# chenhaoxing/DiffUTE

Measured on AMD Instinct MI355X. Metric: 512x512 50-step denoise images/sec, higher is better.
Workload: dtype bf16; 1 GPU; SD2-inpaint UNet 50-step DDIM denoise loop, 512x512 px, batch 4 per GPU, glyph context [B,577,1024], ctx K/V cached per image (BASELINE configs[1]); VAE encode/decode not in the timed region; global_batch=4, denoise_steps=50, parallelism=replicas x1 (no collective), weights=random-init SD2-inpainting shapes (865,925,124 params), bf16 packed

## Files before the change

diffute_amd/_cabi.py:

```python
import ctypes
import os
from ctypes import c_char_p, c_float, c_int, c_int64, c_size_t, c_void_p, POINTER

_LIB_DIR = os.path.join(os.path.dirname(os.path.abspath(__file__)), "lib")
_LIB_PATH = os.environ.get("DIFFUTE_HIP_LIB") or os.path.join(_LIB_DIR, "libdiffute_hip.so")
_LIB_PATH_F16 = os.environ.get("DIFFUTE_HIP_LIB_F16") or os.path.join(_LIB_DIR, "libdiffute_hip_f16.so")
_lib = None
_lib_f16 = None
_exclusive = None
_last_elem = "bf16"


class XfChainDesc(ctypes.Structure):
    _fields_ = [
        ("M", c_int), ("C", c_int), ("x", c_void_p), ("ldx", c_int), ("res", c_void_p), ("ldres", c_int),
        ("w0", c_void_p), ("b0", c_void_p), ("h_out", c_void_p), ("ldh", c_int), ("w1", c_void_p),
        ("c1", c_void_p), ("c2", c_void_p), ("y", c_void_p), ("ldy", c_int), ("wf1", c_void_p),
        ("wf2", c_void_p), ("bf2", c_void_p), ("wpo", c_void_p), ("bpo", c_void_p), ("xres", c_void_p), ("ldxres", c_int),
        ("eps", c_float), ("dbg", c_int), ("timing", c_void_p), ("colstats", c_void_p), ("cs_rows", c_int),
        ("gn_st", c_void_p), ("gn_gamma", c_void_p), ("gn_beta", c_void_p), ("gn_groups", c_int), ("gn_rows", c_int), ("gn_eps", c_float),
    ]


class GemmDesc(ctypes.Structure):
# ... 85 lines not shown
    "dmx_test_transpose_bf16": (c_int, [_P, c_int, _P, c_int, c_int, c_int, _P]),
    "dmx_test_transpose_batch": (c_int, [_P, c_int, _P, c_size_t, _P]),
    "dmx_test_add_bf16": (c_int, [_P, c_int, _P, c_int, _P, c_int, c_int, c_int, _P]),
    "dmx_test_softmax_rows": (c_int, [_P, c_int, _P, c_int, c_int, c_int, c_float, _P]),
    "dmx_test_softmax_bwd_rows": (c_int, [_P, c_int, _P, c_int, _P, c_int, c_int, c_int, c_float, _P]),
    "dmx_test_pointwise_small_fwd": (c_int, [_P, c_int, _P, c_int, _P, _P, c_int, c_int, c_int, c_int, c_int, _P]),
    "dmx_test_pointwise_small_bwd_workspace_bytes": (c_size_t, [c_int, c_int, c_int]),
    "dmx_test_pointwise_small_bwd": (c_int, [_P, c_int, _P, c_int, _P, c_int, _P, c_int, _P, c_int, _P, c_int, c_int, c_int, _P, c_size_t, _P]),
    "dmx_test_linear_small_bwd": (c_int, [_P, c_int, _P, c_int, _P, c_int, _P, c_int, _P, c_int, _P, c_int, c_int, c_int, c_int, c_int, c_int, _P]),
    "dmx_test_slice_cast": (c_int, [_P, c_int, _P, c_int, c_int, c_int, _P]),
    "dmx_test_mode_bwd": (c_int, [_P, c_int, _P, c_int, c_int, _P]),
    "dmx_test_bf16_to_f32_rows": (c_int, [_P, c_int, _P, c_int, c_int, _P]),
    "dmx_conv_gemm_workspace_bytes": (c_size_t, [POINTER(GemmDesc)]),
    "dmx_conv_gemm": (c_int, [POINTER(GemmDesc), _P, c_size_t, _P]),
    "dmx_conv_gemm_rowstats_tiles": (c_int, [POINTER(GemmDesc)]),
    "dmx_conv_gemm_colstats_ok": (c_int, [POINTER(GemmDesc)]),
    "dmx_set_gn_producer_stats": (c_int, [c_int]),
    "dmx_conv3x3_gn_supported": (c_int, [POINTER(HaloConvDesc)]),
    "dmx_conv3x3_gn_workspace_bytes": (c_size_t, [POINTER(HaloConvDesc)]),
    "dmx_conv3x3_gn": (c_int, [POINTER(HaloConvDesc), _P, c_size_t, _P]),
    "dmx_colstats": (c_int, [_P, c_int, c_int, c_int, c_int, _P, _P]),
    "dmx_skinny_conv_supported": (c_int, [POINTER(SkinnyDesc)]),
    "dmx_skinny_conv_workspace_bytes": (c_size_t, [POINTER(SkinnyDesc)]),
    "dmx_skinny_conv": (c_int, [POINTER(SkinnyDesc), _P, c_size_t, _P]),
    "dmx_skinny_pack": (c_int, [_P, c_int, _P, c_int, c_int, POINTER(c_int), POINTER(c_int), POINTER(c_int), POINTER(c_int), _P]),
    "dmx_set_skinny": (c_int, [c_int]),
    "dmx_set_halo_conv": (c_int, [c_int]),
    "dmx_set_halo_ws": (c_int, [c_int]),
    "dmx_set_halo_peers": (c_int, [c_int]),
    "dmx_set_attn_balanced": (c_int, [c_int]),
    "dmx_attention_fwd_v_balanced_workspace_bytes": (c_size_t, [c_int, c_int, c_int, c_int]),
    "dmx_attention_fwd_v_balanced": (c_int, [c_void_p, c_int, c_void_p, c_int, c_void_p, c_int, c_int, c_void_p, c_int, c_int, c_int, c_int, c_int, c_float,
                                             c_void_p, c_size_t, c_void_p]),
    "dmx_set_defer_reduce": (c_int, [c_int]),
    "dmx_set_exclusive_device": (c_int, [c_int]),
    "dmx_get_exclusive_device": (c_int, []),
    "dmx_plan_epoch": (c_int, []),
    "dmx_xf_chain_ok": (c_int, [c_int, c_int]),
    "dmx_xf_chain": (c_int, [POINTER(XfChainDesc), c_int, _P]),
    "dmx_set_xf_chain": (c_int, [c_int]),
    "dmx_set_weight_prefetch": (c_int, [c_int]),
    "dmx_groupnorm_from_stats": (c_int, [_P, c_int, _P, c_int, c_int, c_int, c_int, c_int, c_int, _P, _P, c_float, c_int, _P, _P, _P, c_int, _P]),
    "dmx_conv_wgrad_workspace_bytes": (c_size_t, [POINTER(GemmDesc), c_int]),
    "dmx_conv_wgrad": (c_int, [POINTER(GemmDesc), _P, c_int, _P, c_int, _P, c_size_t, _P]),
    "dmx_colsum_workspace_bytes": (c_size_t, [c_int, c_int, c_int]),
    "dmx_colsum": (c_int, [_P, c_int, c_int, c_int, c_int, _P, c_int, c_int, _P, c_size_t, _P]),
    "dmx_groupnorm_workspace_bytes": (c_size_t, [c_int, c_int, c_int]),
    "dmx_groupnorm": (c_int, [_P, c_int, _P, c_int, c_int, c_int, c_int, c_int, c_int, _P, _P, c_float, c_int, _P, c_int, _P, c_size_t, _P]),
    "dmx_groupnorm_train": (c_int, [_P, c_int, _P, c_int, c_int, c_int, c_int, c_int, c_int, _P, _P, c_float, c_int, _P, c_int, _P, _P, c_size_t, _P]),
    "dmx_groupnorm_bwd_workspace_bytes": (c_size_t, [c_int, c_int, c_int]),
    "dmx_groupnorm_bwd": (c_int, [_P, c_int, _P, c_int, c_int, c_int, c_int, c_int, c_int, _P, _P, c_int, _P,
                                  _P, c_int, _P, c_int, _P, c_int, _P, c_int, _P, c_int, _P, _P, c_int, _P, c_size_t, _P]),
    "dmx_layernorm_bwd_workspace_bytes": (c_size_t, [c_int, c_int]),
    "dmx_layernorm_bwd": (c_int, [_P, c_int, _P, c_int, _P, _P, c_int, _P, c_int, _P, _P, c_int, c_int, c_int, c_float, _P, c_size_t, _P]),
    "dmx_geglu_fwd": (c_int, [_P, c_int, _P, c_int, c_int, c_int, _P]),
    "dmx_geglu_bwd": (c_int, [_P, c_int, _P, c_int, _P, c_int, c_int, c_int, _P]),
    "dmx_layernorm": (c_int, [_P, c_int, _P, c_int, _P, _P, c_int, c_int, c_float, _P]),
    "dmx_attention_fwd": (c_int, [_P, c_int, _P, c_int, c_int, _P, c_int, c_int, _P, c_int, c_int, c_int, c_int, c_int, c_float, _P]),
    "dmx_attention_fwd_v": (c_int, [_P, c_int, _P, c_int, _P, c_int, c_int, _P, c_int, c_int, c_int, c_int, c_int, c_float, _P]),
    "dmx_attention_wide": (c_int, [_P, c_int, _P, c_int, _P, c_int, c_int, _P, c_int, c_int, c_int, c_int, c_int, c_float, _P]),
    "dmx_attention_fwd_train": (c_int, [_P, c_int, _P, c_int, _P, c_int, c_int, _P, c_int, _P, c_int, c_int, c_int, c_int, c_float, _P]),
    "dmx_attention_bwd_workspace_bytes": (c_size_t, [c_int, c_int, c_int]),
    "dmx_attention_bwd": (c_int, [_P, c_int, _P, c_int, _P, c_int, c_int, _P, _P, c_int, _P, _P, c_int, _P, c_int, _P, c_int,
                                  c_int, c_int, c_int, c_int, c_float, _P, c_size_t, _P]),
    "dmx_timestep_embedding": (c_int, [_P, c_int, _P, c_int, c_int, _P, _P]),
    "dmx_linear_small": (c_int, [_P, c_int, _P, c_int, _P, _P, c_int, c_int, c_int, c_int, c_int, _P]),
# ... 235 lines not shown
```

diffute_amd/csrc/attention.hip:

```cpp
#include "common.h"
#include "kernels.h"
#include "attention_d64.h"
#include <stdlib.h>

#define KROW 72
#define VROW 68
#define VRS 192
#define KT_BYTES (64 * KROW * 2)
#define VT_BYTES (64 * VRS)

#define DMX_TR8(V, A, O0, O1, O2, O3, O4, O5, O6, O7)                                                     \
  asm volatile("ds_read_b64_tr_b16 %0, %8 offset:%9\n\tds_read_b64_tr_b16 %1, %8 offset:%10\n\t"          \
               "ds_read_b64_tr_b16 %2, %8 offset:%11\n\tds_read_b64_tr_b16 %3, %8 offset:%12\n\t"         \
               "ds_read_b64_tr_b16 %4, %8 offset:%13\n\tds_read_b64_tr_b16 %5, %8 offset:%14\n\t"         \
               "ds_read_b64_tr_b16 %6, %8 offset:%15\n\tds_read_b64_tr_b16 %7, %8 offset:%16"              \
               : "=&v"(V[0]), "=&v"(V[1]), "=&v"(V[2]), "=&v"(V[3]), "=&v"(V[4]), "=&v"(V[5]), "=&v"(V[6]), "=&v"(V[7]) \
               : "v"(A), "i"(O0), "i"(O1), "i"(O2), "i"(O3), "i"(O4), "i"(O5), "i"(O6), "i"(O7) : "memory")


template <bool VROWMAJOR, int R, int NW, int PROBE = 0>
__global__ __launch_bounds__(64 * NW, R == 2 ? 2 : (NW == 4 ? 2 : 3)) void dmx_attn_d64_kernel(const AttnArgs p) {
  constexpr int NT = 64 * NW, SL = 512 / NT;
  constexpr bool DMA = VROWMAJOR;
  constexpr int KTB = DMA ? 64 * 128 : KT_BYTES, VTB = DMA ? 64 * 128 : VT_BYTES;
// ... 526 lines not shown
    const float inv = 1.0f / l_tot;
    const int qrow = q0 + lr;
#ifdef DMX_ATTN_TIMING
    if (p.lse && lane == 0) {
      float* d = p.lse + ((size_t)((blockIdx.z * gridDim.y + blockIdx.y) * gridDim.x + blockIdx.x) * 4 + wave) * 4;
      d[0] = (float)tm_top; d[1] = (float)tm_slots; d[2] = (float)tm_wait; d[3] = (float)tm_bar;
    }
#else
    if (p.lse && qrow < p.Sq && lh == 0) p.lse[((size_t)b * p.H + h) * p.Sq + qrow] = m_run * sl2 + log2f(l_tot);
#endif
    if (qrow < p.Sq) {
      bf16* op = p.o + ((size_t)b * p.Sq + qrow) * p.ldo + h * 64 + 4 * lh;
#pragma unroll
      for (int dt = 0; dt < 2; ++dt)
#pragma unroll
        for (int g = 0; g < 4; ++g) {
          u32x2 pk = {pack_bf2(o[dt][4 * g] * inv, o[dt][4 * g + 1] * inv),
                      pack_bf2(o[dt][4 * g + 2] * inv, o[dt][4 * g + 3] * inv)};
          *(u32x2*)(op + 32 * dt + 8 * g) = pk;
        }
    }
  }
}

#endif

int dmx_attention_launch(const AttnArgs& a, hipStream_t stream) {
  DMX_REQUIRE(a.B > 0 && a.H > 0 && a.Sq > 0 && a.Skv > 0, "attention: empty problem");
  DMX_REQUIRE(a.kv_rows >= a.Skv, "attention: kv_rows=%d < Skv=%d", a.kv_rows, a.Skv);
  DMX_REQUIRE(a.ldq % 8 == 0 && a.ldk % 8 == 0 && a.ldo % 4 == 0, "attention: strides must be multiples of 8 (ldq=%d ldk=%d)", a.ldq, a.ldk);
  dim3 grid(cdiv(a.Sq, 128), a.H, a.B);
  if (a.v) {
    DMX_REQUIRE(a.ldv % 8 == 0, "attention: ldv=%d must be a multiple of 8", a.ldv);
#ifdef DMX_ATTN_PIPE
#ifndef DMX_ATTN_PIPE_MIN
#define DMX_ATTN_PIPE_MIN 1
#endif
    if (a.Skv >= DMX_ATTN_PIPE_MIN) {
      hipLaunchKernelGGL(dmx_attn_d64_pipe_kernel, grid, dim3(256), 0, stream, a);
      dmx_profile_note_symbol("dmx_attn_d64_pipe_kernel(AttnArgs)");
      return dmx_check_launch("dmx_attn_d64_pipe_kernel");
    }
#endif
#ifdef DMX_PROBES
#define PB(N) else if (pb == N) hipLaunchKernelGGL((dmx_attn_d64_kernel<true, 1, 4, N>), grid, dim3(256), 0, stream, a);
    if (const int pb = getenv("DMX_ATTN_PROBE_BITS") ? atoi(getenv("DMX_ATTN_PROBE_BITS")) : 0; pb == 0) hipLaunchKernelGGL((dmx_attn_d64_kernel<true, 1, 4>), grid, dim3(256), 0, stream, a);
    PB(1) PB(2) PB(4) PB(8) PB(16) PB(32) PB(96) PB(3) PB(7) PB(24) PB(31) PB(127) PB(120)
#undef PB
#else
    hipLaunchKernelGGL((dmx_attn_d64_kernel<true, 1, 4>), grid, dim3(256), 0, stream, a);
#endif
    dmx_profile_note_symbol("void dmx_attn_d64_kernel<true, 1, 4, 0>(AttnArgs)");
  } else {
    grid = dim3(cdiv(a.Sq, 128), a.H, a.B);
    DMX_REQUIRE(a.vt && a.ldvt % 8 == 0 && a.skv_stride % 8 == 0, "attention: V^T strides must be multiples of 8 (ldvt=%d skv_stride=%d)", a.ldvt, a.skv_stride);
    DMX_REQUIRE(a.skv_stride >= (a.Skv + 7) / 8 * 8, "attention: skv_stride=%d < Skv=%d rounded to 8", a.skv_stride, a.Skv);
    hipLaunchKernelGGL((dmx_attn_d64_kernel<false, 1, 4>), grid, dim3(256), 0, stream, a);
  }
  return dmx_check_launch("dmx_attn_d64_kernel");
}
```

diffute_amd/csrc/exec.hip:

```cpp
#include <stdarg.h>
#include <stdio.h>
#include <string.h>
#include "exec.h"
#include <vector>

static thread_local char g_err[512] = "";
void dmx_set_error(const char* fmt, ...) {
  va_list ap; va_start(ap, fmt); vsnprintf(g_err, sizeof(g_err), fmt, ap); va_end(ap);
}
const char* dmx_get_error() { return g_err; }
static int* g_dev_err = nullptr;
int* dmx_dev_err_words() {
  static bool tried = false;
  if (!tried) {
    tried = true;
    void* p = nullptr;
    if (hipHostMalloc(&p, 64, hipHostMallocMapped | hipHostMallocCoherent) == hipSuccess && p) { memset(p, 0, 64); g_dev_err = (int*)p; }
    else (void)hipGetLastError();
  }
  return g_dev_err;
}
int dmx_poll_device_error() {
  volatile int* e = g_dev_err;
  if (!e || !e[0]) return DMX_OK;
  const int k = e[0], blk = e[2], d0 = e[3], d1 = e[4], d2 = e[5];
  if (k == DMX_DEVK_HALO_PEER)
    dmx_set_error("device error: conv3x3_gn (halo conv) block %d gave up after 40 ms waiting for the K-split slab of peer %d of tile slot %d (splits %d) - "
                  "the blocks of a tile were not co-resident (CUs taken by another stream?); the result of that launch is invalid", blk, d1, d0, d2);
  else if (k == DMX_DEVK_STREAMK_HELPER)
    dmx_set_error("device error: stream-K GEMM block %d (tile %d) gave up after 40 ms waiting for the partial sums of helper block %d - "
                  "the blocks of the launch were not co-resident; the result of that launch is invalid", blk, d0, d1);
  else if (k == DMX_DEVK_SKINNY_PEER)
    dmx_set_error("device error: weight-streaming conv (skinny.hip) block %d gave up after 40 ms waiting for the partial tile of K slice %d of output tile %d (slices %d) - "
                  "the blocks of a tile were not co-resident (CUs taken by another stream?); the result of that launch is invalid", blk, d1, d0, d2);
  else if (k == DMX_DEVK_ATTN_PEER)
    dmx_set_error("device error: attention (balanced schedule) slot %d gave up after 40 ms waiting for the partial (O, m, l) record of slot %d for query block %d (%d slots) - "
                  "the slots in front of it did not run; the result of that launch is invalid", blk, d0, d1, d2);
  else
    dmx_set_error("device error %d raised by block %d (%d, %d, %d)", k, blk, d0, d1, d2);
  e[0] = 0;
  for (int i = 2; i < 8; ++i) e[i] = 0;
  __atomic_thread_fence(__ATOMIC_SEQ_CST);
  e[1] = 0;
  return DMX_ERR_DEVICE;
}
extern "C" int dmx_device_error(void) { return dmx_poll_device_error(); }
int dmx_check_launch(const char* what) {
  hipError_t e = hipGetLastError();
  if (e != hipSuccess) { dmx_set_error("launch of %s failed: %s", what, hipGetErrorString(e)); return DMX_ERR_HIP; }
  const int rc = dmx_poll_device_error();
  if (rc) {
    char first[400]; strncpy(first, dmx_get_error(), sizeof(first) - 1); first[sizeof(first) - 1] = 0;
    dmx_set_error("%s [surfaced at the launch check of %s, which itself was enqueued correctly; the walk it belongs to is abandoned]", first, what ? what : "?");
  }
  return rc;
}

static int g_plan_sw[DMX_SW_COUNT] = {1, 1, 1, 1, 1, 1, 1, 0, 1, 1, 1};
void dmx_plan_switch(int slot, int value) { if (slot >= 0 && slot < DMX_SW_COUNT) g_plan_sw[slot] = value; }
void dmx_plan_epoch_bump() { ++g_plan_sw[DMX_SW_OVERRIDES]; }
extern "C" int dmx_plan_epoch(void) {
  unsigned h = 2166136261u;
  for (int i = 0; i < DMX_SW_COUNT; ++i) h = (h ^ (unsigned)g_plan_sw[i]) * 16777619u;
  return (int)(h & 0x7fffffffu);
}

namespace {
struct ProfRec { hipEvent_t a, b; int cls; double flops, bytes; char tag[96]; char sym[112]; };
struct ProfSym { char sym[112]; int cls; double n, ms, flops, bytes; };
std::vector<ProfSym> g_prof_syms;
bool g_prof_on = false;
std::vector<ProfRec> g_prof;
char g_prof_path[512] = "";
}
ProfScope::ProfScope(ProfClass c, hipStream_t s, double flops, double bytes, const char* tag) {
  if (!g_prof_on) return;
  ProfRec r; r.cls = c; r.flops = flops; r.bytes = bytes; r.tag[0] = 0; r.sym[0] = 0;
  if (tag) { strncpy(r.tag, tag, sizeof(r.tag) - 1); r.tag[sizeof(r.tag) - 1] = 0; }
  if (hipEventCreate(&r.a) != hipSuccess || hipEventCreate(&r.b) != hipSuccess) return;
  (void)hipEventRecord(r.a, s);
  slot = (int)g_prof.size(); g_prof.push_back(r);
  stream_ = s;
}
ProfScope::~ProfScope() { if (slot >= 0) (void)hipEventRecord(g_prof[slot].b, stream_); }

bool dmx_profile_active() { return g_prof_on; }
void dmx_profile_note_symbol(const char* sym) {
  if (!g_prof_on || g_prof.empty() || !sym) return;
  strncpy(g_prof.back().sym, sym, sizeof(g_prof.back().sym) - 1); g_prof.back().sym[sizeof(g_prof.back().sym) - 1] = 0;
}
extern "C" int dmx_profile_begin(void) {
// ... 473 lines not shown
static int g_xf_chain = 1;
extern "C" int dmx_set_xf_chain(int on) { const int old = g_xf_chain; g_xf_chain = on; dmx_plan_switch(DMX_SW_XF_CHAIN, on); return old; }
bool Exec::chain_ok(const Tn& x) const { return (g_xf_chain & 3) && !f32 && x.ld == x.C && ((g_xf_chain & 3) > 1 ? dmx_xf_chain_supported(x.rows(), x.C) : dmx_xf_chain_pays(x.rows(), x.C)); }
bool Exec::chain_gn_fold(const Tn& x) const { return !(g_xf_chain & 4) && !f32 && x.cst != nullptr && (x.H * x.W) % 64 == 0 && x.ld == x.C; }
void Exec::chain_stats(XfChainArgs& a, Tn& y) {
  if (rc || f32 || !dmx_halo_conv_enabled() || !g_gn_producer_stats || (y.H * y.W) % 64) return;
  if (!dmx_conv_halo_wants_stats(y.H, y.W, g_halo_conv != 1)) return;
  a.colstats = stat_slice(y.B, y.C);
  if (!a.colstats) return;
  a.cs_rows = y.H * y.W; y.cst = a.colstats;
}
void Exec::xf_chain(int mode, XfChainArgs& a) {
  const long cc = (long)a.C * a.C * 2;
  note(a.w0, cc);
  if (mode == 0) note(a.w1, cc);
  else if (mode == 2) note(a.w1, 3 * cc);
  else { note(a.wf1, 8 * cc); note(a.wf2, 4 * cc); note(a.wpo, cc); }
  peek(a.pf, a.pf_bytes, 4);
  if (dry || rc) return;
  rc = dmx_xf_chain_launch(a, mode, stream);
}

void Exec::attention(const bf16* q, int ldq, const bf16* k, int ldk, const bf16* v, int ldv, int kv_rows,
                     bf16* o, int ldo, int B, int H, int Sq, int Skv, float scale, bool kv_static) {
#ifdef DMX_PROBES
  static const int kv_pf = [] { const char* e = getenv("DMX_PF_KV"); return e ? atoi(e) : 1; }();
#else
  constexpr int kv_pf = 1;
#endif
  if (kv_static && kv_pf) note(k, (long)B * kv_rows * ldk * 2);
  AttnArgs a{};
  a.q = q; a.ldq = ldq; a.k = k; a.ldk = ldk; a.kv_rows = kv_rows; a.v = v; a.ldv = ldv;
  a.o = o; a.ldo = ldo; a.B = B; a.H = H; a.Sq = Sq; a.Skv = Skv; a.scale = scale;
  const int sk_slots = f32 ? 0 : dmx_attention_balanced_slots(a);
  void* sk_ws = nullptr;
  if (sk_slots) {
    constexpr size_t POOL = 64 * 1024;
    if (!flag_pool) {
      flag_pool = (int*)raw(POOL * sizeof(int)); flag_cap = POOL; flag_used = 0;
      if (!zero_pool(flag_pool, POOL * sizeof(int), 2)) return;
    }
    const size_t n = align_up((size_t)sk_slots, 64);
    const size_t pb = dmx_attention_balanced_part_bytes(a);
    if (flag_used + n <= flag_cap) { a.sk_flags = flag_pool + flag_used; flag_used += n; sk_ws = raw(pb); a.sk_part = (float*)sk_ws; }
  }
  struct Rel { Workspace& w; void* p; ~Rel() { if (p) w.release(p); } } rel{ws, sk_ws};
  if (dry || rc) return;
  if (f32) {
    rc = dmx_attention_f32_launch((const float*)q, ldq, (const float*)k, ldk, (const float*)v, ldv, kv_rows, (float*)o, ldo, B, H, Sq, Skv, scale, stream);
    return;
  }
  {
#ifdef DMX_PROBES
    static const int attn_pf = [] { const char* e = getenv("DMX_PF_ATTN"); return e ? atoi(e) : 1; }();
#else
    constexpr int attn_pf = 1;
#endif
    if (attn_pf) peek(a.pf, a.pf_bytes, 4);
  }
  char tag[96]; snprintf(tag, sizeof(tag), "B=%d H=%d Sq=%d Skv=%d", B, H, Sq, Skv);
  ProfScope ps(PROF_ATTN, stream, 4.0 * B * H * (double)Sq * Skv * 64.0, 2.0 * 64.0 * B * H * (2.0 * Sq + 2.0 * Skv), tag);
  rc = a.sk_part ? dmx_attention_balanced_launch(a, stream) : dmx_attention_launch(a, stream);
}

void Exec::tap(const Tn& t) {
  if (!taps) return;
  flush(t);
// ... 88 lines not shown
```

diffute_amd/csrc/kernels.h:

```cpp
#pragma once
#include <vector>
#include "common.h"

enum ProfClass { PROF_GEMM128 = 0, PROF_GEMM64 = 1, PROF_SPLITK = 2, PROF_ATTN = 3, PROF_GNORM = 4, PROF_LNORM = 5,
                 PROF_OTHER = 6, PROF_GEMM256 = 7, PROF_WGRAD = 8, PROF_GEMM256WS = 9,
                 PROF_GEMM_CFG0 = 10 , PROF_XFCHAIN = 26 , PROF_HALO = 27 , PROF_SKINNY = 28 , PROF_NCLASS = 29 };
int n_cus();
enum DmxPlanSwitch { DMX_SW_EXCLUSIVE = 0, DMX_SW_GN_STATS, DMX_SW_DEFER, DMX_SW_HALO, DMX_SW_PREFETCH, DMX_SW_XF_CHAIN, DMX_SW_HALO_WS, DMX_SW_OVERRIDES, DMX_SW_SKINNY, DMX_SW_HALO_PEERS, DMX_SW_ATTN_BALANCED, DMX_SW_COUNT };
void dmx_plan_switch(int slot, int value);
void dmx_plan_epoch_bump();
extern "C" int dmx_plan_epoch(void);
int dmx_exclusive_device();
void dmx_profile_note_symbol(const char* sym);
struct ProfScope {
  ProfScope(ProfClass c, hipStream_t s, double flops, double bytes, const char* tag = nullptr);
  ~ProfScope();
  int slot = -1;
  hipStream_t stream_ = nullptr;
};

struct GemmArgs {
  const bf16* x0; const bf16* x1;
  int ldx0, ldx1;
  int cx0;
  int direct;
  int IH, IW, OH, OW;
  int stride, pad, ups, ksize;
  int ups2, M4; long long w_phase_stride;
  int Cin;
  int Ktaps;
  const bf16* s0; const bf16* s1; int lds0, lds1, cs0;
  const bf16* w; int ldw;
  int M, N, K;
  const float* bias;
  const float* rowbias;
  int rows_per_group, ldrb;
  const bf16* res; int ldres;
  void* out; int ldo; int out_f32; int geglu;
  int act;
  int force_tn, force_splitk;
  int group_m;
// ... 171 lines not shown
  bf16* y; int ldy;
  const bf16* wf1;
  const bf16* wf2; const float* bf2;
  const bf16* wpo; const float* bpo;
  const bf16* xres; int ldxres;
  float eps;
  int dbg; long long* timing;
  long long* colstats; int cs_rows;
  const void* pf[4]; int pf_bytes[4];
  const long long* gn_st; const float* gn_gamma; const float* gn_beta; int gn_groups; int gn_rows; float gn_eps;
};
bool dmx_xf_chain_supported(int M, int C);
bool dmx_xf_chain_pays(int M, int C);
int dmx_xf_chain_launch(const XfChainArgs& a, int mode, hipStream_t stream);

struct AttnArgs {
  const bf16* q; int ldq;
  const bf16* k; int ldk;
  int kv_rows;
  const bf16* vt; int ldvt;
  const bf16* v; int ldv;
  int skv_stride;
  bf16* o; int ldo;
  int B, H, Sq, Skv;
  float scale;
  float* lse;
  const void* pf[4]; int pf_bytes[4];
  float* sk_part; int* sk_flags; int* err;
};
int dmx_attention_launch(const AttnArgs& a, hipStream_t stream);
int dmx_attention_balanced_slots(const AttnArgs& a);
size_t dmx_attention_balanced_part_bytes(const AttnArgs& a);
int dmx_attention_balanced_launch(AttnArgs a, hipStream_t stream);

struct AttnWideArgs {
  const bf16* q; int ldq;
  const bf16* k; int ldk;
  const bf16* v; int ldv;
  int kv_rows;
  bf16* o; int ldo;
  int B, Sq, Skv, D;
  float scale;
  const bf16* zeros;
};
bool dmx_attention_wide_supported(int D);
int dmx_attention_wide_launch(AttnWideArgs a, hipStream_t stream);

struct AttnBwdArgs {
  const bf16* q; int ldq; const bf16* k; int ldk; const bf16* v; int ldv; int kv_rows;
  const bf16* o; const bf16* dout; int ldo;
  const float* lse;
  float* delta;
  bf16* dq; int lddq; bf16* dk; int lddk; bf16* dv; int lddv;
  int B, H, Sq, Skv; float scale;
};
size_t dmx_attn_bwd_ws_bytes(int B, int H, int Sq);
int dmx_attention_bwd_launch(const AttnBwdArgs& a, hipStream_t stream);

struct GemmF32Args {
  const float* x0; const float* x1; int ldx0, ldx1, cx0, direct;
  int IH, IW, OH, OW, stride, pad, ups, ksize, Cin, Ktaps;
  const float* s0; const float* s1; int lds0, lds1, cs0;
  const float* w; int ldw; int M, N, K;
  const float* bias; const float* bias2; const float* rowbias; int rows_per_group, ldrb;
  const float* res; int ldres;
  float* out; int ldo; int geglu, act;
// ... 72 lines not shown
```

include/diffute_hip.h:

```cpp
#ifndef DIFFUTE_HIP_H
#define DIFFUTE_HIP_H

#include <stddef.h>
#include <stdint.h>

#ifdef __cplusplus
extern "C" {
#endif

#define DMX_OK 0
#define DMX_ERR_ARG (-1)
#define DMX_ERR_HIP (-2)
#define DMX_ERR_UNSUPPORTED (-3)
#define DMX_ERR_WORKSPACE (-4)

typedef void* dmx_stream_t;
typedef struct dmx_unet dmx_unet;
typedef struct dmx_vae dmx_vae;

int dmx_version(void);
const char* dmx_last_error(void);
int dmx_device_error(void);
int dmx_test_raise_device_error(int code, dmx_stream_t stream);
int dmx_test_occupy_cus(int blocks, long long ticks, dmx_stream_t stream);
const char* dmx_element_type(void);

int dmx_test_transpose_bf16(const void* in, int ldin, void* out, int ldout, int R, int C, dmx_stream_t stream);
typedef struct dmx_test_tr_job { const void* in; int ldin; void* out; int ldout; int R, C; } dmx_test_tr_job;
int dmx_test_transpose_batch(const dmx_test_tr_job* h_jobs, int njobs, void* table, size_t table_bytes, dmx_stream_t stream);
int dmx_test_add_bf16(const void* a, int lda, const void* b, int ldb, void* out, int ldo, int rows, int C, dmx_stream_t stream);
int dmx_test_softmax_rows(const float* s, int lds, void* p, int ldp, int rows, int n, float scale, dmx_stream_t stream);
int dmx_test_softmax_bwd_rows(const void* p, int ldp, const float* dp, int lddp, void* ds, int ldds, int rows, int n, float scale, dmx_stream_t stream);
int dmx_test_pointwise_small_fwd(const void* x, int ldx, const void* w, int ldw, const float* bias, void* y, int ldy, int M, int Cin, int Cout,
                                 int out_f32, dmx_stream_t stream);
size_t dmx_test_pointwise_small_bwd_workspace_bytes(int M, int Cin, int Cout);
int dmx_test_pointwise_small_bwd(const void* x, int ldx, const float* dy, int lddy, const void* w, int ldw, void* dx, int lddx,
                                 float* dw, int lddw, float* db, int M, int Cin, int Cout, void* workspace, size_t workspace_bytes, dmx_stream_t stream);
int dmx_test_linear_small_bwd(const float* x, int ldx, const float* dy, int lddy, const void* w, int ldw, float* dw, int lddw, float* db, int db_stride,
                              float* dx, int lddx, int B, int N, int K, int silu_in, int accumulate, dmx_stream_t stream);
int dmx_test_slice_cast(const float* in, int ldin, void* out, int ldo, int M, int C, dmx_stream_t stream);
int dmx_test_mode_bwd(const void* dz, int lddz, float* dmom, int M, int C, dmx_stream_t stream);
int dmx_test_bf16_to_f32_rows(const void* in, int ldin, float* out, int M, int C, dmx_stream_t stream);


typedef struct dmx_gemm_desc {
  const void* x0; const void* x1;
  int ldx0, ldx1, cx0;
  int direct;
  int IH, IW, OH, OW;
  int stride, pad, ups, ksize;
  int Cin;
  int Ktaps;
  const void* s0; const void* s1;
  int lds0, lds1, cs0;
  const void* w; int ldw;
  int M, N, K;
  const float* bias;
  const float* rowbias;
  int rows_per_group, ldrb;
  const void* res; int ldres;
  void* out; int ldo; int out_f32;
  int geglu;
  int force_tn, force_splitk;
  int group_m;
  long long* timing;
  int dbg;
  int act;
  float* rowstats_out;
  const float* ln_stats; int ln_tiles;
  const float* ln_c1; const float* ln_c2; int ln_C; float ln_eps;
  long long* colstats; int cs_rows;
} dmx_gemm_desc;
size_t dmx_conv_gemm_workspace_bytes(const dmx_gemm_desc* d);
int dmx_set_gn_producer_stats(int on);
int dmx_conv_gemm_colstats_ok(const dmx_gemm_desc* d);
// ... 104 lines not shown

int dmx_groupnorm_train(const void* x0, int ldx0, const void* x1, int ldx1, int c0, int C, int groups,
                        int B, int HW, const float* gamma, const float* beta, float eps, int silu,
                        void* y, int ldy, float* stats, void* workspace, size_t workspace_bytes, dmx_stream_t stream);
size_t dmx_groupnorm_bwd_workspace_bytes(int B, int HW, int C);
int dmx_groupnorm_bwd(const void* x0, int ldx0, const void* x1, int ldx1, int c0, int C, int groups, int B, int HW,
                      const float* gamma, const float* beta, int silu, const float* stats,
                      const void* dy, int lddy, void* dx0, int lddx0, void* dx1, int lddx1,
                      const void* res0, int ldres0, const void* res1, int ldres1,
                      float* dgamma, float* dbeta, int accumulate,
                      void* workspace, size_t workspace_bytes, dmx_stream_t stream);
size_t dmx_layernorm_bwd_workspace_bytes(int rows, int C);
int dmx_layernorm_bwd(const void* x, int ldx, const void* dy, int lddy, const float* gamma, void* dx, int lddx,
                      const void* res, int ldres, float* dgamma, float* dbeta, int accumulate,
                      int rows, int C, float eps, void* workspace, size_t workspace_bytes, dmx_stream_t stream);
int dmx_geglu_fwd(const void* h, int ldh, void* y, int ldy, int rows, int C2, dmx_stream_t stream);
int dmx_geglu_bwd(const void* h, int ldh, const void* dy, int lddy, void* dh, int lddh, int rows, int C2, dmx_stream_t stream);

int dmx_layernorm(const void* x, int ldx, void* y, int ldy, const float* gamma, const float* beta,
                  int rows, int C, float eps, dmx_stream_t stream);

int dmx_attention_fwd(const void* q, int ldq, const void* k, int ldk, int kv_rows,
                      const void* vt, int ldvt, int skv_stride, void* o, int ldo,
                      int B, int H, int Sq, int Skv, float scale, dmx_stream_t stream);

int dmx_attention_wide(const void* q, int ldq, const void* k, int ldk, const void* v, int ldv, int kv_rows,
                       void* o, int ldo, int B, int Sq, int Skv, int D, float scale, dmx_stream_t stream);
int dmx_attention_fwd_v(const void* q, int ldq, const void* k, int ldk, const void* v, int ldv, int kv_rows,
                        void* o, int ldo, int B, int H, int Sq, int Skv, float scale, dmx_stream_t stream);
size_t dmx_attention_fwd_v_balanced_workspace_bytes(int B, int H, int Sq, int Skv);
int dmx_attention_fwd_v_balanced(const void* q, int ldq, const void* k, int ldk, const void* v, int ldv, int kv_rows,
                                 void* o, int ldo, int B, int H, int Sq, int Skv, float scale,
                                 void* workspace, size_t workspace_bytes, dmx_stream_t stream);
int dmx_set_attn_balanced(int mode);

int dmx_attention_fwd_train(const void* q, int ldq, const void* k, int ldk, const void* v, int ldv, int kv_rows,
                            void* o, int ldo, float* lse, int B, int H, int Sq, int Skv, float scale, dmx_stream_t stream);
size_t dmx_attention_bwd_workspace_bytes(int B, int H, int Sq);
int dmx_attention_bwd(const void* q, int ldq, const void* k, int ldk, const void* v, int ldv, int kv_rows,
                      const void* o, const void* d_o, int ldo, const float* lse,
                      void* dq, int lddq, void* dk, int lddk, void* dv, int lddv,
                      int B, int H, int Sq, int Skv, float scale,
                      void* workspace, size_t workspace_bytes, dmx_stream_t stream);

int dmx_timestep_embedding(const int64_t* t, int t_count, const float* freq, int B, int dim, float* out, dmx_stream_t stream);
int dmx_linear_small(const float* x, int ldx, const void* w_bf16, int ldw, const float* bias, float* y, int ldy,
                     int B, int N, int K, int silu_in, dmx_stream_t stream);

int dmx_im2col_small(const float* f0, int c0, const float* f1, int c1, const float* f2, int c2,
                     const void* h_nhwc, int ldh, int C, int B, int IH, int IW, int OH, int OW,
                     int ksize, int stride, int pad, void* out, int Kpad, dmx_stream_t stream);

int dmx_pack_conv_weight(const float* w, void* out, int Cout, int Cin, int ksize, int ldk, int koff, dmx_stream_t stream);
int dmx_pack_linear_weight(const float* w, void* out, int rows, int cols, int ldo, int geglu, dmx_stream_t stream);
int dmx_pack_geglu_bias(const float* b, float* out, int n, dmx_stream_t stream);
int dmx_pack_conv_weight_t(const float* w, void* out, int Cout, int Cin, int ksize, int ldk, int koff, dmx_stream_t stream);
int dmx_pack_linear_weight_t(const float* w, void* out, int rows, int cols, int ldo, dmx_stream_t stream);
int dmx_zero_insert2(const void* dy, int lddy, void* z, int B, int OH, int OW, int C, dmx_stream_t stream);
int dmx_sumpool2(const void* du, int lddu, int du_f32, void* dx, int lddx, int B, int H, int W, int C, int accumulate, dmx_stream_t stream);

int dmx_cast_f32_to_bf16(const float* in, void* out, size_t n, dmx_stream_t stream);
int dmx_nhwc_bf16_to_nchw_f32(const void* in, int ldin, float* out, int B, int C, int HW, dmx_stream_t stream);
int dmx_nhwc_f32_to_nchw_f32(const float* in, int ldin, float* out, int B, int C, int HW, dmx_stream_t stream);
int dmx_nchw_f32_to_nhwc_bf16(const float* in, void* out, int ldo, int B, int C, int HW, dmx_stream_t stream);

int dmx_sched_step_ddim(const float* sample, const float* model_output, const float* noise, float* prev_sample, size_t n,
// ... 293 lines not shown
```

Before: 11.83 images/s.

## Add LDS-resident K/V attention kernel for short cross-attention contexts

```diff
diff --git a/diffute_amd/_cabi.py b/diffute_amd/_cabi.py
--- a/diffute_amd/_cabi.py
+++ b/diffute_amd/_cabi.py
@@ -141,6 +141,11 @@
     "dmx_attention_fwd_v_balanced_workspace_bytes": (c_size_t, [c_int, c_int, c_int, c_int]),
     "dmx_attention_fwd_v_balanced": (c_int, [c_void_p, c_int, c_void_p, c_int, c_void_p, c_int, c_int, c_void_p, c_int, c_int, c_int, c_int, c_int, c_float,
                                              c_void_p, c_size_t, c_void_p]),
+    "dmx_set_attn_resident": (c_int, [c_int]),
+    "dmx_test_attention_resident": (c_int, [c_void_p, c_int, c_void_p, c_int, c_void_p, c_int, c_int, c_void_p, c_int, c_int, c_int, c_int, c_int, c_float,
+                                            c_int, c_void_p]),
+    "dmx_attention_resident_plan": (c_int, [c_int, c_int, c_int, c_int, c_int, c_int, POINTER(c_int), POINTER(c_int), POINTER(c_int)]),
+    "dmx_attention_resident_wave_units": (None, [c_int, c_int, c_int, POINTER(c_int), POINTER(c_int)]),
     "dmx_set_defer_reduce": (c_int, [c_int]),
     "dmx_set_exclusive_device": (c_int, [c_int]),
     "dmx_get_exclusive_device": (c_int, []),
diff --git a/diffute_amd/csrc/attention.hip b/diffute_amd/csrc/attention.hip
--- a/diffute_amd/csrc/attention.hip
+++ b/diffute_amd/csrc/attention.hip
@@ -582,6 +582,7 @@
   dim3 grid(cdiv(a.Sq, 128), a.H, a.B);
   if (a.v) {
     DMX_REQUIRE(a.ldv % 8 == 0, "attention: ldv=%d must be a multiple of 8", a.ldv);
+    if (dmx_attention_resident_blocks(a)) return dmx_attention_resident_launch(a, stream);
 #ifdef DMX_ATTN_PIPE
 #ifndef DMX_ATTN_PIPE_MIN
 #define DMX_ATTN_PIPE_MIN 1
diff --git a/diffute_amd/csrc/attention_res.hip b/diffute_amd/csrc/attention_res.hip
--- /dev/null
+++ b/diffute_amd/csrc/attention_res.hip
@@ -0,0 +1,252 @@
+#include "common.h"
+#include "kernels.h"
+#include "attention_d64.h"
+
+template <bool TAIL>
+__device__ __forceinline__ void res_tile(const char* ks, const char* vs, const int kv0, const int Skv, const int ns4_tail, const bf16x8 (&qf)[4],
+                                         f32x16 (&o)[2], float& m_run, float& l_run, const float sl2, const int lane) {
+  const int ns4 = TAIL ? ns4_tail : 4;
+  const int lr = lane & 31, lh = lane >> 5;
+  const int ksw = (lh ^ ((lr >> 1) & 7)) << 4;
+  f32x16 s[2];
+  const f32x16 zero = {0.f, 0.f, 0.f, 0.f, 0.f, 0.f, 0.f, 0.f, 0.f, 0.f, 0.f, 0.f, 0.f, 0.f, 0.f, 0.f};
+  if (!TAIL) {
+    bf16x8 kf[2][4];
+#pragma unroll
+    for (int kk = 0; kk < 4; ++kk)
+#pragma unroll
+      for (int kt = 0; kt < 2; ++kt) kf[kt][kk] = *(const bf16x8*)(ks + (32 * kt + lr) * 128 + (((2 * kk) << 4) ^ ksw));
+#pragma unroll
+    for (int kk = 0; kk < 4; ++kk)
+#pragma unroll
+      for (int kt = 0; kt < 2; ++kt) s[kt] = DMX_MFMA_32x32x16(kf[kt][kk], qf[kk], kk == 0 ? zero : s[kt]);
+    __builtin_amdgcn_sched_group_barrier(0x100, 8, 0);
+    __builtin_amdgcn_sched_group_barrier(0x008, 8, 0);
+  } else {
+#pragma unroll
+    for (int kt = 0; kt < 2; ++kt) {
+#pragma unroll
+      for (int r = 0; r < 16; ++r) s[kt][r] = -INFINITY;
+      if (2 * kt < ns4) {
+        bf16x8 kf[4];
+#pragma unroll
+        for (int kk = 0; kk < 4; ++kk) kf[kk] = *(const bf16x8*)(ks + (32 * kt + lr) * 128 + (((2 * kk) << 4) ^ ksw));
+#pragma unroll
+        for (int kk = 0; kk < 4; ++kk) s[kt] = DMX_MFMA_32x32x16(kf[kk], qf[kk], kk == 0 ? zero : s[kt]);
+#pragma unroll
+        for (int r = 0; r < 16; ++r) {
+          const int key = kv0 + 32 * kt + (r & 3) + 8 * (r >> 2) + 4 * lh;
+          if (key >= Skv) s[kt][r] = -INFINITY;
+        }
+      }
+    }
+  }
+  bf16x8 pf[4];
+  auto exponentiate = [&](float mc) {
+    float q0 = 0.f, q1 = 0.f;
+#pragma unroll
+    for (int kt = 0; kt < 2; ++kt)
+#pragma unroll
+      for (int u = 0; u < 2; ++u) {
+        if (TAIL && 2 * kt + u >= ns4) { pf[2 * kt + u] = __builtin_bit_cast(bf16x8, (u32x4){0u, 0u, 0u, 0u}); continue; }
+        unsigned int w[4];
+#pragma unroll
+        for (int e = 0; e < 4; ++e) {
+          const float a0 = __builtin_fmaf(s[kt][8 * u + 2 * e], sl2, mc), a1 = __builtin_fmaf(s[kt][8 * u + 2 * e + 1], sl2, mc);
+          const float p0 = __builtin_amdgcn_exp2f(a0), p1 = __builtin_amdgcn_exp2f(a1);
+          q0 += p0; q1 += p1;
+          w[e] = pack_bf2(p0, p1);
+        }
+        u32x4 wv = {w[0], w[1], w[2], w[3]};
+        pf[2 * kt + u] = __builtin_bit_cast(bf16x8, wv);
+      }
+    return q0 + q1;
+  };
+  float psum = exponentiate(-m_run * sl2);
+  if (__any(!(psum <= 8192.0f))) {
+    float mx = -INFINITY;
+#pragma unroll
+    for (int kt = 0; kt < 2; ++kt)
+#pragma unroll
+      for (int r = 0; r < 16; ++r) mx = fmaxf(mx, s[kt][r]);
+    mx = fmaxf(mx, __shfl_xor(mx, 32));
+    const float m_new = fmaxf(m_run, mx);
+    const float alpha = __builtin_amdgcn_exp2f((m_run - m_new) * sl2);
+    m_run = m_new;
+    l_run *= alpha;
+#pragma unroll
+    for (int i = 0; i < 16; ++i) { o[0][i] *= alpha; o[1][i] *= alpha; }
+    psum = exponentiate(-m_run * sl2);
+  }
+  l_run += psum;
+
+  const int p16 = lane & 15, g = lane >> 4;
+  const char* va = vs + (4 * (g >> 1) + (p16 >> 2)) * 128 + (16 * (g & 1) + 4 * (p16 & 3)) * 2;
+  const int vsw = (p16 >> 3) & 1;
+#pragma unroll
+  for (int dt = 0; dt < (TAIL ? 1 : 2); ++dt)
+#pragma unroll
+    for (int s4 = 0; s4 < 4; ++s4) {
+      if (TAIL) {
+        if (s4 < ns4) {
+#pragma unroll
+          for (int d2 = 0; d2 < 2; ++d2) {
+            const s16x4 lo = __builtin_amdgcn_ds_read_tr16_b64_v4i16((lds_s16x4)(va + 64 * (d2 ^ vsw) + (2 * s4) * 8 * 128));
+            const s16x4 hi = __builtin_amdgcn_ds_read_tr16_b64_v4i16((lds_s16x4)(va + 64 * (d2 ^ vsw) + (2 * s4 + 1) * 8 * 128));
+            const s16x8 vv = __builtin_shufflevector(lo, hi, 0, 1, 2, 3, 4, 5, 6, 7);
+            o[d2] = DMX_MFMA_32x32x16(__builtin_bit_cast(bf16x8, vv), pf[s4], o[d2]);
+          }
+        }
+        continue;
+      }
+      const s16x4 lo = __builtin_amdgcn_ds_read_tr16_b64_v4i16((lds_s16x4)(va + 64 * (dt ^ vsw) + (2 * s4) * 8 * 128));
+      const s16x4 hi = __builtin_amdgcn_ds_read_tr16_b64_v4i16((lds_s16x4)(va + 64 * (dt ^ vsw) + (2 * s4 + 1) * 8 * 128));
+      const s16x8 vv = __builtin_shufflevector(lo, hi, 0, 1, 2, 3, 4, 5, 6, 7);
+      o[dt] = DMX_MFMA_32x32x16(__builtin_bit_cast(bf16x8, vv), pf[s4], o[dt]);
+    }
+}
+
+__host__ __device__ static inline void res_wave_units(int nu, int nw_pair, int w, int* u0, int* u1) {
+  *u0 = (int)((long long)w * nu / nw_pair); *u1 = (int)((long long)(w + 1) * nu / nw_pair);
+}
+
+template <int NW>
+__global__ __launch_bounds__(64 * NW, 1) void dmx_attn_d64_res_kernel(const AttnArgs p) {
+  extern __shared__ __attribute__((aligned(16))) char res_smem[];
+  const int t = threadIdx.x, lane = t & 63, wave = __builtin_amdgcn_readfirstlane(t >> 6);
+  const int lr = lane & 31, lh = lane >> 5;
+  const int b = blockIdx.z, h = blockIdx.y;
+  const float sl2 = p.scale * 1.4426950408889634f;
+  const int rows = (p.Skv + 31) & ~31;
+  char* kimg = res_smem;
+  char* vimg = kimg + rows * 128;
+  char* dump = vimg + rows * 128;
+
+  int u0, u1;
+  const int nu = (p.Sq + 31) >> 5;
+  res_wave_units(nu, gridDim.x * NW, blockIdx.x * NW + wave, &u0, &u1);
+
+  bf16x8 qf[4];
+  auto load_q = [&](int u) {
+    int qrow = 32 * u + lr; if (qrow >= p.Sq) qrow = p.Sq - 1;
+    const bf16* qp = p.q + ((size_t)b * p.Sq + qrow) * p.ldq + h * 64 + 8 * lh;
+#pragma unroll
+    for (int kk = 0; kk < 4; ++kk) qf[kk] = *(const bf16x8*)(qp + 16 * kk);
+  };
+  load_q(u0 < nu ? u0 : nu - 1);
+
+  {
+    const int drow = lane >> 3, dchk = lane & 7;
+    const unsigned ldkb = (unsigned)p.ldk * 2u, ldvb = (unsigned)p.ldv * 2u;
+    const unsigned vcb = (unsigned)((((((dchk >> 2) ^ ((drow >> 1) & 1)) << 2) | (dchk & 3))) << 4);
+    const char* kdma = (const char*)(p.k + (size_t)b * p.kv_rows * p.ldk + h * 64);
+    const char* vdma = (const char*)(p.v + (size_t)b * p.kv_rows * p.ldv + h * 64);
+    const int nslab = rows >> 3, last = p.Skv - 1;
+    for (int s = wave; s < nslab; s += NW) {
+      const unsigned rc = (unsigned)min(8 * s + drow, last);
+      const unsigned kcb = (unsigned)((dchk ^ (((drow >> 1) + 4 * (s & 1)) & 7)) << 4);
+      dmx_dma16((kdma + (size_t)rc * ldkb + kcb), DMX_LDS_ADDR((kimg + s * 1024)));
+    }
+    for (int s = wave; s < nslab; s += NW) {
+      const unsigned rc = (unsigned)min(8 * s + drow, last);
+      dmx_dma16((vdma + (size_t)rc * ldvb + vcb), DMX_LDS_ADDR((vimg + s * 1024)));
+    }
+  }
+  asm volatile("s_waitcnt vmcnt(0)" ::: "memory");
+#pragma unroll
+  for (int kk = 0; kk < 4; ++kk) asm volatile("" : "+v"(qf[kk]));
+  {
+    const int nblk = gridDim.x * gridDim.y * gridDim.z, blk = (blockIdx.z * gridDim.y + blockIdx.y) * gridDim.x + blockIdx.x;
+    int npf = 0;
+#pragma unroll
+    for (int r = 0; r < 4; ++r) {
+      const int nb = p.pf_bytes[r];
+      for (int u = blk * NW + wave; u * 1024 < nb && npf < 3; u += nblk * NW, ++npf) {
+        int off = u * 1024 + lane * 16; if (off > nb - 16) off = nb - 16;
+        dmx_dma16(((const char*)p.pf[r] + off), DMX_LDS_ADDR(dump));
+      }
+    }
+  }
+  asm volatile("s_waitcnt lgkmcnt(0)" ::: "memory");
+  __builtin_amdgcn_s_barrier();
+  __builtin_amdgcn_sched_barrier(0);
+
+  const int nfull = p.Skv >> 6, rem = p.Skv & 63;
+  for (int u = u0; u < u1; ++u) {
+    if (u != u0) {
+      load_q(u);
+#pragma unroll
+      for (int kk = 0; kk < 4; ++kk) asm volatile("" : "+v"(qf[kk]));
+    }
+    f32x16 o[2];
+#pragma unroll
+    for (int i = 0; i < 16; ++i) { o[0][i] = 0.f; o[1][i] = 0.f; }
+    float m_run = -INFINITY, l_run = 0.f;
+
+    for (int it = 0; it < nfull; ++it) res_tile<false>(kimg + it * 8192, vimg + it * 8192, it * 64, p.Skv, 4, qf, o, m_run, l_run, sl2, lane);
+    if (rem) res_tile<true>(kimg + nfull * 8192, vimg + nfull * 8192, nfull * 64, p.Skv, (rem + 15) >> 4, qf, o, m_run, l_run, sl2, lane);
+
+    const float l_tot = l_run + __shfl_xor(l_run, 32);
+    const float inv = 1.0f / l_tot;
+    const int qrow = 32 * u + lr;
+    if (qrow < p.Sq) {
+      bf16* op = p.o + ((size_t)b * p.Sq + qrow) * p.ldo + h * 64 + 4 * lh;
+#pragma unroll
+      for (int dt = 0; dt < 2; ++dt)
+#pragma unroll
+        for (int g = 0; g < 4; ++g) {
+          u32x2 pk = {pack_bf2(o[dt][4 * g] * inv, o[dt][4 * g + 1] * inv),
+                      pack_bf2(o[dt][4 * g + 2] * inv, o[dt][4 * g + 3] * inv)};
+          *(u32x2*)(op + 32 * dt + 8 * g) = pk;
+        }
+    }
+  }
+  asm volatile("s_waitcnt vmcnt(0)" ::: "memory");
+}
+
+static int g_attn_resident = 1;
+extern "C" int dmx_set_attn_resident(int mode) { const int old = g_attn_resident; g_attn_resident = mode; dmx_plan_switch(DMX_SW_ATTN_RESIDENT, mode); return old; }
+
+#define RES_MAX_SKV 608
+#define RES_MIN_UPB 9
+extern "C" int dmx_attention_resident_plan(int B, int H, int Sq, int Skv, int cus, int mode, int* blocks_per_pair, int* waves, int* lds_bytes) {
+  if (blocks_per_pair) *blocks_per_pair = 0;
+  if (waves) *waves = 0;
+  if (lds_bytes) *lds_bytes = 0;
+  if (mode <= 0 || B <= 0 || H <= 0 || Sq <= 0 || Skv <= 0 || Skv > RES_MAX_SKV || cus <= 0) return 0;
+  const long long pairs = (long long)B * H;
+  const int nu = cdiv(Sq, 32);
+  int nbp = pairs >= cus ? 1 : (int)(cus / pairs);
+  if (nbp > nu) nbp = nu;
+  const int upb = cdiv(nu, nbp);
+  if (mode == 1 && (pairs > cus || upb < RES_MIN_UPB || upb > 12)) return 0;
+  const int nw = upb <= 4 ? 4 : (upb <= 8 ? 8 : 12);
+  if (blocks_per_pair) *blocks_per_pair = nbp;
+  if (waves) *waves = nw;
+  if (lds_bytes) *lds_bytes = 2 * ((Skv + 31) & ~31) * 128 + 1024;
+  return nbp;
+}
+extern "C" void dmx_attention_resident_wave_units(int nu, int waves_per_pair, int w, int* u0, int* u1) { res_wave_units(nu, waves_per_pair, w, u0, u1); }
+
+int dmx_attention_resident_blocks(const AttnArgs& a) {
+  if (!a.v || a.lse) return 0;
+  return dmx_attention_resident_plan(a.B, a.H, a.Sq, a.Skv, n_cus(), g_attn_resident, nullptr, nullptr, nullptr);
+}
+
+template <int NW>
+static int res_launch(const AttnArgs& a, int nbp, int lds, hipStream_t stream) {
+  DMX_LDS_OPT_IN(dmx_attn_d64_res_kernel<NW>, 2 * RES_MAX_SKV * 128 + 1024);
+  hipLaunchKernelGGL((dmx_attn_d64_res_kernel<NW>), dim3(nbp, a.H, a.B), dim3(64 * NW), lds, stream, a);
+  return DMX_OK;
+}
+int dmx_attention_resident_launch(const AttnArgs& a, hipStream_t stream, int cus) {
+  int nbp = 0, nw = 0, lds = 0;
+  DMX_REQUIRE(cus >= 0 && cus <= n_cus(), "attention (resident K/V): plan for %d CUs on a device with %d", cus, n_cus());
+  if (a.v && !a.lse) dmx_attention_resident_plan(a.B, a.H, a.Sq, a.Skv, cus ? cus : n_cus(), cus ? 2 : g_attn_resident, &nbp, &nw, &lds);
+  DMX_REQUIRE(nbp > 0, "attention (resident K/V): not planned for B=%d H=%d Sq=%d Skv=%d", a.B, a.H, a.Sq, a.Skv);
+  DMX_REQUIRE(a.ldq % 8 == 0 && a.ldk % 8 == 0 && a.ldv % 8 == 0 && a.ldo % 4 == 0 && a.kv_rows >= a.Skv, "attention (resident K/V): strides");
+  if (nw == 4) { if (const int rc = res_launch<4>(a, nbp, lds, stream)) return rc; dmx_profile_note_symbol("void dmx_attn_d64_res_kernel<4>(AttnArgs)"); }
+  else if (nw == 8) { if (const int rc = res_launch<8>(a, nbp, lds, stream)) return rc; dmx_profile_note_symbol("void dmx_attn_d64_res_kernel<8>(AttnArgs)"); }
+  else { if (const int rc = res_launch<12>(a, nbp, lds, stream)) return rc; dmx_profile_note_symbol("void dmx_attn_d64_res_kernel<12>(AttnArgs)"); }
+  return dmx_check_launch("dmx_attn_d64_res_kernel");
+}
diff --git a/diffute_amd/csrc/exec.hip b/diffute_amd/csrc/exec.hip
--- a/diffute_amd/csrc/exec.hip
+++ b/diffute_amd/csrc/exec.hip
@@ -56,7 +56,7 @@
   return rc;
 }
 
-static int g_plan_sw[DMX_SW_COUNT] = {1, 1, 1, 1, 1, 1, 1, 0, 1, 1, 1};
+static int g_plan_sw[DMX_SW_COUNT] = {1, 1, 1, 1, 1, 1, 1, 0, 1, 1, 1, 1};
 void dmx_plan_switch(int slot, int value) { if (slot >= 0 && slot < DMX_SW_COUNT) g_plan_sw[slot] = value; }
 void dmx_plan_epoch_bump() { ++g_plan_sw[DMX_SW_OVERRIDES]; }
 extern "C" int dmx_plan_epoch(void) {
@@ -596,7 +596,7 @@
   AttnArgs a{};
   a.q = q; a.ldq = ldq; a.k = k; a.ldk = ldk; a.kv_rows = kv_rows; a.v = v; a.ldv = ldv;
   a.o = o; a.ldo = ldo; a.B = B; a.H = H; a.Sq = Sq; a.Skv = Skv; a.scale = scale;
-  const int sk_slots = f32 ? 0 : dmx_attention_balanced_slots(a);
+  const int sk_slots = f32 || dmx_attention_resident_blocks(a) ? 0 : dmx_attention_balanced_slots(a);
   void* sk_ws = nullptr;
   if (sk_slots) {
     constexpr size_t POOL = 64 * 1024;
diff --git a/diffute_amd/csrc/kernels.h b/diffute_amd/csrc/kernels.h
--- a/diffute_amd/csrc/kernels.h
+++ b/diffute_amd/csrc/kernels.h
@@ -6,7 +6,7 @@
                  PROF_OTHER = 6, PROF_GEMM256 = 7, PROF_WGRAD = 8, PROF_GEMM256WS = 9,
                  PROF_GEMM_CFG0 = 10 , PROF_XFCHAIN = 26 , PROF_HALO = 27 , PROF_SKINNY = 28 , PROF_NCLASS = 29 };
 int n_cus();
-enum DmxPlanSwitch { DMX_SW_EXCLUSIVE = 0, DMX_SW_GN_STATS, DMX_SW_DEFER, DMX_SW_HALO, DMX_SW_PREFETCH, DMX_SW_XF_CHAIN, DMX_SW_HALO_WS, DMX_SW_OVERRIDES, DMX_SW_SKINNY, DMX_SW_HALO_PEERS, DMX_SW_ATTN_BALANCED, DMX_SW_COUNT };
+enum DmxPlanSwitch { DMX_SW_EXCLUSIVE = 0, DMX_SW_GN_STATS, DMX_SW_DEFER, DMX_SW_HALO, DMX_SW_PREFETCH, DMX_SW_XF_CHAIN, DMX_SW_HALO_WS, DMX_SW_OVERRIDES, DMX_SW_SKINNY, DMX_SW_HALO_PEERS, DMX_SW_ATTN_BALANCED, DMX_SW_ATTN_RESIDENT, DMX_SW_COUNT };
 void dmx_plan_switch(int slot, int value);
 void dmx_plan_epoch_bump();
 extern "C" int dmx_plan_epoch(void);
@@ -244,6 +244,8 @@
 int dmx_attention_balanced_slots(const AttnArgs& a);
 size_t dmx_attention_balanced_part_bytes(const AttnArgs& a);
 int dmx_attention_balanced_launch(AttnArgs a, hipStream_t stream);
+int dmx_attention_resident_blocks(const AttnArgs& a);
+int dmx_attention_resident_launch(const AttnArgs& a, hipStream_t stream, int cus = 0);
 
 struct AttnWideArgs {
   const bf16* q; int ldq;
diff --git a/include/diffute_hip.h b/include/diffute_hip.h
--- a/include/diffute_hip.h
+++ b/include/diffute_hip.h
@@ -41,6 +41,8 @@
 int dmx_test_slice_cast(const float* in, int ldin, void* out, int ldo, int M, int C, dmx_stream_t stream);
 int dmx_test_mode_bwd(const void* dz, int lddz, float* dmom, int M, int C, dmx_stream_t stream);
 int dmx_test_bf16_to_f32_rows(const void* in, int ldin, float* out, int M, int C, dmx_stream_t stream);
+int dmx_test_attention_resident(const void* q, int ldq, const void* k, int ldk, const void* v, int ldv, int kv_rows, void* o, int ldo,
+                                int B, int H, int Sq, int Skv, float scale, int cus, dmx_stream_t stream);
 
 
 typedef struct dmx_gemm_desc {
@@ -211,6 +213,9 @@
 int dmx_attention_fwd_v_balanced(const void* q, int ldq, const void* k, int ldk, const void* v, int ldv, int kv_rows,
                                  void* o, int ldo, int B, int H, int Sq, int Skv, float scale,
                                  void* workspace, size_t workspace_bytes, dmx_stream_t stream);
+int dmx_set_attn_resident(int mode);
+int dmx_attention_resident_plan(int B, int H, int Sq, int Skv, int cus, int mode, int* blocks_per_pair, int* waves, int* lds_bytes);
+void dmx_attention_resident_wave_units(int units, int waves_per_pair, int w, int* u0, int* u1);
 int dmx_set_attn_balanced(int mode);
 
 int dmx_attention_fwd_train(const void* q, int ldq, const void* k, int ldk, const void* v, int ldv, int kv_rows,
```

Result: no change. 11.82 images/s (-0.1%).
